# fishaudio/Bert-VITS2

Hardware: AMD Instinct MI355X
Metric: audio-seconds/sec (44.1 kHz), SynthesizerTrn.infer(), 128-phoneme utterance (higher is better)
Workload: dtype f32; 1 GPU; BASELINE config 2: B=1 x T=128 symbols per GPU, fp32 Generator (split-bf16 MFMA), fp32 flow, fp32 text encoder / durations / spline; utterances_per_gpu=1, symbols=128, frames=384, parallelism=utterance-sharded x1, hipgraph=False, hip_force_dev_kernarg=1

## Files before the change

### bert-vits2_amd/csrc/bv2_api.cpp

```cpp
#include <cmath>
#include <cstddef>
#include <cstring>
#include <functional>
#include <new>

#include "bv2_internal.h"

using namespace bv2;

static thread_local std::string g_create_err;

#define BV2_TRY try {
#define BV2_CATCH(h_)                                                                  \
  } catch (const std::exception& e) {                                                  \
    if (h_) (h_)->err = std::string("exception: ") + e.what();                         \
    return -100;                                                                       \
  } catch (...) {                                                                      \
    if (h_) (h_)->err = "unknown exception";                                           \
    return -100;                                                                       \
  }

extern "C" {

int bv2_abi_version(void) { return BV2_ABI_VERSION; }
// ... 459 lines not shown
}

int bv2_graph_num_nodes(const bv2_graph* g) { return g ? g->nodes : -1; }

void bv2_graph_destroy(bv2_graph* g) {
  if (!g) return;
  if (g->exec) (void)hipGraphExecDestroy(g->exec);
  delete g;
}

int bv2_set_option(bv2_handle* h, const char* key, int value) {
  if (!h) return -1;
  BV2_TRY
  const std::string k = key ? key : "";
  if (k == "fused_resblock") h->no_fused_resblock = value == 0;
  else if (k == "fused_respair") h->no_fused_respair = value == 0;
  else if (k == "fused_boundary") h->no_fused_boundary = value == 0;
  else if (k == "x6_pair") h->no_x6_pair = value == 0;
  else if (k == "x6_pair_c64") h->no_x6_pair_c64 = value == 0;
  else if (k == "x6_pair_c16") h->no_x6_pair_c16 = value == 0;
  else if (k == "x6_pair_c128") h->x6_pair_c128 = value != 0;
  else if (k == "respair_mix") h->respair_problem_major = value == 0;
  else if (k == "respair_form") h->respair_form = value;
  else if (k == "respair_c32") h->no_respair_c32 = value == 0;
  else if (k == "f16_wn") h->f16_wn = value;
  else if (k == "f16_ni") h->f16_ni = value;
  else if (k == "f16_kv") h->no_f16_kv = !value;
  else if (k == "stage_sum") h->no_stage_sum = !value;
  else if (k == "resblock_c16") h->no_resblock_c16 = value == 0;
  else if (k == "f16_fused_ln") h->no_f16_fused_ln = value == 0;
  else if (k == "f16_ksplit") h->no_f16_ksplit = value == 0;
  else if (k == "conv_post_rows") h->no_conv_post_rows = value == 0;
  else if (k == "ups_phase_taps") h->no_ups_phase_taps = value == 0;
  else if (k == "xcd_affine") h->no_xcd_affine = value == 0;
  else if (k == "prefetch") h->prefetch = value & 3;
  else if (k == "conv_x6") h->no_conv_x6 = value == 0;
  else if (k == "conv_x3") h->no_conv_x3 = value == 0;
  else if (k == "conv_x6_c32") h->x6_narrow = value != 0;
  else if (k == "fused_dds") h->no_fused_dds = value == 0;
  else if (k == "fused_attn_o") h->no_fused_attn_o = value == 0;
  else if (k == "attn_ksplit") h->attn_ksplit = value;
  else if (k == "overlap_dp") h->no_overlap_dp = value == 0;
  else { h->err = "bv2_set_option: unknown key '" + k + "'"; return -1; }
  return 0;
  BV2_CATCH(h)
}

int bv2_set_tap(bv2_handle* h, const char* name, float* dev_dst, int64_t cap) {
  if (!h) return -1;
  BV2_TRY
  if (!name) { h->taps.clear(); return 0; }
  if (!dev_dst || cap <= 0) { h->taps.erase(name); return 0; }
  h->taps[name] = Tap{dev_dst, cap};
  return 0;
  BV2_CATCH(h)
}

int bv2_profile_enable(bv2_handle* h, int on) {
  if (!h) return -1;
  BV2_TRY
  if (on && h->prof_pool.empty()) {
    h->prof_pool.resize(8192);
    for (auto& r : h->prof_pool) {
      if (hipEventCreate(&r.e0) != hipSuccess || hipEventCreate(&r.e1) != hipSuccess) {
        h->err = "bv2_profile_enable: hipEventCreate failed";
        return -6;
// ... 135 lines not shown
            std::memcpy(&wy[x3_w_index(j, ci, co, cin, k, 0)], &g0, 2);
            std::memcpy(&wy[x3_w_index(j, ci, co, cin, k, 1)], &g1, 2);
          }
    }
    if (w_host && hipMemcpy(wpack_dev, pk.data(), sizeof(float) * pk.size(), hipMemcpyHostToDevice) != hipSuccess) return -6;
    ConvLaunch cl;
    std::memset(&cl, 0, sizeof(cl));
    ConvProb& p = cl.p[0];
    if (cin % 32 == 0 && ksplit <= 1) {
      float* reg = wpack_dev + t_x3_off(cin, cout, k);
      if (launch_x3_zero_slots(static_cast<hipStream_t>(stream), reinterpret_cast<unsigned*>(reg), 2)) return -6;
      p.omax = reinterpret_cast<unsigned*>(reg + X3_SLOT_WORDS);
      if (x3) {
        if (nsrc != 1 || launch_absmax(static_cast<hipStream_t>(stream), x, (int64_t)B * cin * L, reinterpret_cast<unsigned*>(reg))) return -2;
        p.xmax = reinterpret_cast<const unsigned*>(reg);
        p.w3inv = reg + 2 * X3_SLOT_WORDS; p.w3 = reinterpret_cast<const uint16_t*>(reg + 2 * X3_SLOT_WORDS + X3_HDR_FLOATS);
      }
    }
    p.x[0] = x; p.x[1] = x1; p.x[2] = x2; p.nsrc = nsrc; p.in_scale = in_scale;
    p.x_bstride = (int64_t)cin * L; p.x_rstride = L; p.Lin = L;
    p.in_mask = in_mask; p.in_mask_bstride = L; p.out_mask = out_mask; p.out_mask_bstride = L;
    p.w = wpack_dev; p.bias = bias_host ? wpack_dev + boff : nullptr;
    if (x6) p.w6 = reinterpret_cast<const uint16_t*>(wpack_dev + t_x6_off(cin, cout, k));
    p.bias2 = bias2; p.bias2_bstride = cout;
    p.out = out; p.out_bstride = (int64_t)cout * L; p.out_rstride = L; p.out_tstride = 1; p.out_toff = 0;
    p.res = res; p.res_bstride = p.out_bstride; p.res_mode = res_mode;
    p.cin = cin; p.cin_pad = cin_pad; p.cout = cout; p.cout_pad = cout_pad; p.w_ld = ld; p.k = k; p.dil = dil;
    p.pad_left = pad_left < 0 ? ((k - 1) / 2) * dil : pad_left;
    p.pre_act = lrelu_slope != 0.f ? PRE_LRELU : PRE_NONE; p.slope = lrelu_slope;
    p.act = relu ? ACT_RELU : ACT_NONE; p.mask_pre = mask_pre; p.mask_post = mask_post;
    cl.nprob = 1; cl.B = B; cl.L = L; cl.ksplit = ksplit < 1 ? 1 : ksplit; cl.slab_stride = slab_stride;
    const char* vn = nullptr;
    return launch_conv1d(static_cast<hipStream_t>(stream), cl, tile, &vn);
  } catch (...) { return -100; }
}

int bv2_test_resblock_fused(void* stream, const float* x, float* out, const float* w1_host, const float* b1_host,
                            const float* w2_host, const float* b2_host, float* wpack_dev, int B, int C, int k, int dil, int L,
                            float slope) {
  try {
    const int cin_pad = t_round_up(C, 16);
    const size_t one = (size_t)bv2_test_conv_pack_floats(C, C, k), boff = (size_t)k * cin_pad * t_round_up(C, 128);
    std::vector<float> pk(2 * one, 0.f);
    const float* ws[2] = {w1_host, w2_host};
    const float* bs[2] = {b1_host, b2_host};
    for (int h = 0; h < 2; ++h) {
      for (int j = 0; j < k; ++j)
        for (int ci = 0; ci < C; ++ci)
          for (int co = 0; co < C; ++co)
            pk[h * one + (size_t)conv_w_index(j, ci, co, cin_pad, k)] = ws[h][((size_t)co * C + ci) * k + j];
      for (int co = 0; co < C; ++co) pk[h * one + boff + co] = bs[h][co];
    }
    if (hipMemcpy(wpack_dev, pk.data(), sizeof(float) * pk.size(), hipMemcpyHostToDevice) != hipSuccess) return -6;
    FusedLaunch F;
    std::memset(&F, 0, sizeof(F));
    F.nprob = 1; F.B = B; F.C = C; F.L = L; F.slope = slope;
    F.p[0].x = x; F.p[0].out = out; F.p[0].w1 = wpack_dev; F.p[0].b1 = wpack_dev + boff;
    F.p[0].w2 = wpack_dev + one; F.p[0].b2 = wpack_dev + one + boff; F.p[0].k = k; F.p[0].dil = dil;
    return launch_resblock_fused(static_cast<hipStream_t>(stream), F);
  } catch (...) { return -100; }
}

static inline uint16_t t_f2bf(float f) {
  uint32_t u;
  std::memcpy(&u, &f, 4);
  u += 0x7fffu + ((u >> 16) & 1u);
// ... 436 lines not shown
```

### bert-vits2_amd/csrc/bv2_exec.cpp

```cpp
#include <cmath>
#include <cstdlib>
#include <cstring>

#include "bv2_internal.h"

namespace bv2 {

namespace {

struct Arena {
  char* base;
  int64_t off = 0, cap;
  Arena(void* b, int64_t c) : base(static_cast<char*>(b)), cap(c) {}
  template <class T> T* get(int64_t n) {
    const int64_t bytes = (n * (int64_t)sizeof(T) + 255) / 256 * 256;
    T* p = base ? reinterpret_cast<T*>(base + off) : nullptr;
    off += bytes;
    return p;
  }
  bool ok() const { return base == nullptr || off <= cap; }
};

struct Ctx {
  bv2_handle* h;
// ... 743 lines not shown
        if (!last) {
          ConvProb r = c.prob(K.wn_res[i], P.acts, P.h, Ty);
          r.res = P.h; r.res_mode = RES_ADD; r.out_mask = ymask; r.mask_post = 1;
          cl.p[cl.nprob++] = r;
        }
        ConvProb sk = c.prob(K.wn_skip[i], P.acts, P.outacc, Ty);
        if (i > 0) { sk.res = P.outacc; sk.res_mode = RES_ADD; }
        if (last) { sk.out_mask = ymask; sk.mask_post = 1; }
        cl.p[cl.nprob++] = sk;
        c.conv(cl, "wn.res_skip");
      }
      hres = P.outacc;
    }
    {
      const std::string tn = "flow." + std::to_string(a) + ".enc";
      c.tap(tn.c_str(), hres, (int64_t)B * H * Ty);
    }
    p = c.prob(K.post, hres, x1, Ty);
    p.out_bstride = (int64_t)C * Ty; p.res = x1; p.res_bstride = (int64_t)C * Ty; p.res_mode = RES_RSUB;
    p.out_mask = ymask; p.mask_post = 1;
    c.conv1(p, B, Ty, "flow.post");
    {
      const std::string tn = "flow." + std::to_string(a) + ".z";
      c.tap(tn.c_str(), z, (int64_t)B * C * Ty);
    }
  }
}

static void gen_core(Ctx& c, const PlanB& P, const float* z, int z_rstride, const float* ymask, int B, int L, float* o,
                     const int64_t* lens) {
  const Model& m = c.m;
  const bv2_config& cf = m.cfg;
  const int C = cf.inter_channels, c0 = cf.upsample_initial_channel;
  {
    ConvProb p = c.prob(m.conv_pre, z, P.pre, L);
    p.x_bstride = (int64_t)C * z_rstride; p.x_rstride = z_rstride; p.Lin = L;
    p.in_mask = ymask; p.in_mask_bstride = z_rstride;
    p.bias2 = P.gv; p.bias2_bstride = P.gv_stride;
    c.conv1(p, B, L, "dec.conv_pre", 1, 0, lens, 1);
  }
  c.tap("dec.pre", P.pre, (int64_t)B * c0 * L);
  const float* src[3] = {P.pre, nullptr, nullptr};
  int nsrc = 1;
  int Lc = L;
  int up = 1;
  int next_slot = 0;
  int n_slots = 0;
  for (int i = 0; i < m.n_ups && !c.h->no_conv_x3 && !c.h->no_conv_x6; ++i)
    if (m.ups[i].cout % 128 == 0 && m.rb[i][0][0][0].wy_off >= 0) n_slots += 1 + 2 * m.n_rbk * m.n_rbd;
  const bool any_x3 = n_slots > 0;
  if (any_x3 && !c.rc) c.chk(launch_x3_zero_slots(c.s, P.xslots, n_slots), "dec.x3_slots");
  for (int i = 0; i < m.n_ups; ++i) {
    const UpW& U = m.ups[i];
    float* const* S = P.set[i & 1];
    float* x = S[0];
    const int Lo = Lc * U.u;
    const int nb = m.n_rbk;
    const bool rb2 = m.rb_type == 2;
    bool fused = U.cout <= 32 && nb <= 3 && !c.h->no_fused_resblock && !rb2;
    bool x6pair = !rb2 && nb <= 3 && !c.h->no_fused_resblock && !c.h->no_conv_x6 && !c.h->no_x6_pair &&
                  (U.cout == 32 || (U.cout == 16 && !c.h->no_x6_pair_c16) || (U.cout == 64 && !c.h->no_x6_pair_c64) ||
                   (U.cout == 128 && c.h->x6_pair_c128));
    for (int j = 0; j < nb && x6pair; ++j)
      for (int d = 0; d < m.n_rbd && x6pair; ++d)
        x6pair = m.rb[i][j][d][0].wx_off >= 0 && m.rb[i][j][d][1].wx_off >= 0 && m.rb[i][j][d][0].k == m.rb[i][j][d][1].k &&
                 respair_x6_supported(U.cout, cf.resblock_kernel_sizes[j], cf.resblock_dilation_sizes[j][d]);
    if (x6pair) fused = true;
    if (fused && !x6pair && c.h->x6_narrow && !c.h->no_conv_x6 && U.cout == 32 && m.rb[i][0][0][0].wx_off >= 0) fused = false;
    for (int j = 0; j < nb && fused && !x6pair; ++j)
      for (int d = 0; d < m.n_rbd; ++d)
        fused = fused && resblock_fused_supported(U.cout, cf.resblock_kernel_sizes[j], cf.resblock_dilation_sizes[j][d]);
    bool x3 = any_x3 && !rb2 && !fused && U.cout % 128 == 0;
    for (int j = 0; j < nb && x3; ++j)
      for (int d = 0; d < m.n_rbd && x3; ++d) x3 = m.rb[i][j][d][0].wy_off >= 0 && m.rb[i][j][d][1].wy_off >= 0;
    unsigned* const slot_x = x3 ? P.xslots + X3_SLOT_WORDS * next_slot++ : nullptr;
    {
      ConvLaunch cl;
      cl.nprob = U.u; cl.B = B; cl.L = Lc; cl.lens = lens; cl.len_mul = up;
      for (int ph = 0; ph < U.u; ++ph) {
        ConvProb p = c.prob(U.phase[ph], src[0], x, Lc);
        p.x[1] = src[1]; p.x[2] = src[2]; p.nsrc = nsrc; p.in_scale = 1.f / (float)nsrc;
        p.pre_act = PRE_LRELU; p.slope = 0.1f;
        p.pad_left = U.pad_left[ph];
        p.out_bstride = (int64_t)U.cout * Lo; p.out_rstride = Lo; p.out_tstride = U.u; p.out_toff = ph;
        p.omax = slot_x;
        cl.p[ph] = p;
      }
      c.conv(cl, "dec.ups");
    }
    {
      const std::string tn = "dec.ups." + std::to_string(i);
      c.tap(tn.c_str(), x, (int64_t)B * U.cout * Lo);
    }
    float* branch_out[BV2_MAX_RESBLOCK_KERNELS];
    if (rb2) {
      for (int d = 0; d < m.n_rbd; ++d) {
        ConvLaunch c1;
        c1.nprob = nb; c1.B = B; c1.L = Lo; c1.lens = lens; c1.len_mul = up * U.u;
        const bool to_cur = ((m.n_rbd - 1 - d) & 1) == 0;
        for (int jj = 0; jj < nb; ++jj) {
          const int j = nb - 1 - jj;
          float* cur = S[1 + j];
          float* tmp = S[1 + nb + j];
          const float* xin = d == 0 ? x : (to_cur ? tmp : cur);
          ConvProb p = c.prob(m.rb[i][j][d][0], xin, to_cur ? cur : tmp, Lo, cf.resblock_dilation_sizes[j][d]);
          p.pre_act = PRE_LRELU; p.slope = 0.1f;
          p.res = xin; p.res_mode = RES_ADD;
          p.w6 = (!c.h->no_conv_x6 && m.rb[i][j][d][0].wx_off >= 0) ? reinterpret_cast<const uint16_t*>(c.W(m.rb[i][j][d][0].wx_off)) : nullptr;
          c1.p[jj] = p;
        }
        c.conv(c1, "dec.resblock2.conv");
// ... 404 lines not shown
```

### bert-vits2_amd/csrc/bv2_internal.h

```cpp
#pragma once
#include <hip/hip_runtime_api.h>
#include <stdint.h>

#include <map>
#include <string>
#include <vector>

#include "../../include/bv2.h"
#include "bv2_kernels.h"

namespace bv2 {

constexpr int kAttnWindow = 4;
constexpr int kCondLayer = 2;
constexpr int kSdpLayers = 3;
constexpr int kSdpKernel = 3;
constexpr int kSdpBins = 10;
constexpr int kSdpFlowsUsed = 3;
constexpr int kDpFilter = 256;
constexpr int kDpKernel = 3;
constexpr int kFlowKernel = 5;
constexpr int kMaxLayers = 16;
constexpr int kMaxFlows = 8;
constexpr uint32_t kBlobMagic = 0x32765642u;
// ... 81 lines not shown
  int post_c = 0, post_k = 7;
  int total_up = 1;
  int64_t total_floats = 0;
  uint32_t cfg_hash = 0;
};

struct HostTensor { std::vector<float> data; std::vector<int64_t> shape; };

struct ProfileRec { hipEvent_t e0, e1; int fam; double flops, bytes; };

struct Tap { float* dst; int64_t cap; };

}

struct bv2_handle {
  bv2::Model model;
  std::map<std::string, bv2::HostTensor> tensors;
  const float* blob = nullptr;
  std::string err;
  std::map<std::string, bv2::Tap> taps;
  int gen_dtype = BV2_F32;
  int flow_dtype = BV2_F32;
  bool no_conv_x6 = false;
  bool no_conv_x3 = false;
  bool x6_narrow = true;
  bool no_fused_resblock = false;
  int prefetch = 0;
  bool no_xcd_affine = false;
  bool no_f16_fused_ln = false;
  int f16_wn = 0, f16_ni = 0;
  bool no_f16_kv = false;
  bool no_f16_ksplit = false;
  bool no_conv_post_rows = false;
  bool no_ups_phase_taps = false;
  bool no_stage_sum = true;
  bool no_resblock_c16 = false;
  bool no_respair_c32 = false;
  int respair_form = 1;
  bool respair_problem_major = false;
  bool x6_pair_c128 = false;
  bool no_x6_pair_c16 = false;
  bool no_x6_pair_c64 = false;
  bool no_x6_pair = false;
  bool no_fused_boundary = false;
  bool no_fused_respair = false;
  bool no_fused_attn_o = false;
  int attn_ksplit = -1;
  bool no_fused_dds = false;
  bool no_overlap_dp = true;
  hipStream_t side_stream = nullptr;
  hipEvent_t ev_fork = nullptr, ev_join = nullptr;
  bool prof_on = false;
  int prof_mode = 1;
  std::vector<bv2::ProfileRec> prof_pool;
  size_t prof_used = 0;
  std::vector<std::string> prof_names;
};

namespace bv2 {

int build_layout(Model& m, std::string& err);
int pack_blob(const Model& m, const std::map<std::string, HostTensor>& t, float* blob, std::string& err);
bool key_in_schema(const Model& m, const std::string& key);

int64_t workspace_bytes(const Model& m, int B, int T, int Ty);
int run_encode(bv2_handle* h, hipStream_t s, const bv2_encode_in& in, const bv2_encode_out& out, void* ws, int64_t wsb,
// ... 20 lines not shown
```

### bert-vits2_amd/csrc/bv2_kernels.h

```cpp
#pragma once
#include <hip/hip_runtime_api.h>
#include <stdint.h>
#include <map>
#include <mutex>
#include <utility>

namespace bv2 {

#if defined(__HIPCC__)
__device__ __forceinline__ bool xcd_decode(unsigned id, int per, int B, int& b, int& r) {
  const unsigned slot = id >> 3;
  b = (int)(slot / (unsigned)per) * 8 + (int)(id & 7u);
  r = (int)(slot % (unsigned)per);
  return b < B;
}
#endif
inline int xcd_grid(int B, int per) { return 8 * ((B + 7) / 8) * per; }

struct Prefetch { const void* ptr; unsigned bytes; };
constexpr int PF_BLOCKS = 128;
#if defined(__HIPCC__)
__device__ __forceinline__ void prefetch_tail(const Prefetch pf, unsigned l, unsigned j, unsigned tid, unsigned nthreads) {
  const unsigned lines = (pf.bytes + 127u) >> 7;
  const unsigned lx = (lines + 7u) >> 3;
// ... 42 lines not shown
  const float* bias2;
  int bias2_bstride;
  float* out;
  int64_t out_bstride;
  int out_rstride, out_tstride, out_toff;
  const float* res;
  int64_t res_bstride;
  const float* out_mask;
  int out_mask_bstride;
  int cin, cin_pad, cout, cout_pad, w_ld, k, dil, pad_left;
  int pre_act;  float slope;
  int act;
  int mask_pre;
  int res_mode;
  int mask_post;
  const uint16_t* w3;
  const float* w3inv;
  const unsigned* xmax;
  unsigned* omax;
};

#define BV2_MAX_PROBS 8
#define BV2_MAX_KSPLIT 8
struct ConvLaunch {
  ConvProb p[BV2_MAX_PROBS];
  int nprob;
  int B;
  int L;
  const int64_t* lens = nullptr; int len_mul = 1;
  int ksplit;
  int64_t slab_stride;
  unsigned long long* dbg = nullptr;
  Prefetch pf = {nullptr, 0};
};
void conv_set_timeline(unsigned long long* dev_buf, long long capacity_u64);
int conv_timeline_report(long long* meta, int max_launches);
unsigned long long* timeline_slice(unsigned gx, unsigned gy, unsigned gz, int tile, int ks, int cin, int L);

enum { TILE_AUTO = 0, TILE_128x128 = 1, TILE_64x128 = 2, TILE_64x64 = 3, TILE_32x128 = 4, TILE_32x256 = 5, TILE_SPLITK = 6, TILE_128x64 = 7,
       TILE_X6 = 8,
       TILE_X6_128x64 = 9, TILE_X6_128x64_LD = 10, TILE_X6_64x128 = 11, TILE_X6_32x256 = 12,
       TILE_X3 = 14 };
int launch_conv1d(hipStream_t stream, const ConvLaunch& L, int tile, const char** variant_name);
inline int64_t x6_w_index(int j, int ci, int co, int cin, int k, int plane) {
  const int64_t U = (int64_t)(cin / 16) * k, u = (int64_t)(ci / 16) * k + j;
  const int lane = (co & 31) + 32 * ((ci % 16) / 8);
  return ((((int64_t)(co >> 5) * U + u) * 3 + plane) * 64 + lane) * 8 + (ci % 8);
}
inline int64_t x6_w_elems(int cin, int cout_pad, int k) { return (int64_t)(cout_pad / 32) * (cin / 16) * k * 3 * 512; }
inline void x6_split(float v, uint16_t h[3]) {
  for (int p = 0; p < 3; ++p) {
    uint32_t u;
    __builtin_memcpy(&u, &v, 4);
    uint16_t b;
    if ((u & 0x7fffffffu) > 0x7f800000u) b = (uint16_t)((u >> 16) | 0x40u);
    else if (p == 0 && (u & 0x7fffffffu) > 0x7f7f0000u) b = (uint16_t)((u >> 16) & 0x8000u) | 0x7f7fu;
    else { u += 0x7fffu + ((u >> 16) & 1u); b = (uint16_t)(u >> 16); }
    h[p] = b;
    const uint32_t w = (uint32_t)b << 16;
    float f;
    __builtin_memcpy(&f, &w, 4);
    v -= f;
  }
}
inline int64_t x3_w_index(int j, int ci, int co, int cin, int k, int plane) {
  const int64_t U = (int64_t)(cin / 16) * k, u = (int64_t)(ci / 16) * k + j;
// ... 343 lines not shown
```

### bert-vits2_amd/csrc/kernels/conv_mfma.hip

```cpp
#include <hip/hip_runtime.h>
#include "../bv2_kernels.h"

namespace bv2 {

typedef float f32x16 __attribute__((ext_vector_type(16)));
typedef float f32x4 __attribute__((ext_vector_type(4)));

__device__ __forceinline__ unsigned* x3_slot_word(unsigned* slot) {
  return slot + X3_LINE_WORDS * (__builtin_amdgcn_s_getreg((31 << 11) | 20) & 7u);
}
__device__ __forceinline__ void x3_publish(unsigned* word, unsigned seen, float vmx, int lane) {
#pragma unroll
  for (int d = 32; d >= 1; d >>= 1) vmx = fmaxf(vmx, __shfl_xor(vmx, d));
  const unsigned bits = __float_as_uint(vmx);
  if (lane == 0 && bits > seen) __hip_atomic_fetch_max(word, bits, __ATOMIC_RELAXED, __HIP_MEMORY_SCOPE_WORKGROUP);
}

__device__ __forceinline__ float ld_off(const float* base, unsigned byte_off) {
  return *reinterpret_cast<const float*>(reinterpret_cast<const char*>(base) + byte_off);
}
__device__ __forceinline__ f32x4 ld_off4(const float* base, unsigned byte_off) {
  return *reinterpret_cast<const f32x4*>(reinterpret_cast<const char*>(base) + byte_off);
}

// ... 280 lines not shown
        }
      }
    }
    if (omax_w) x3_publish(omax_w, omax_seen, vmx, lane);
  }
  if (L.dbg && tid == 0) {
    __builtin_amdgcn_s_waitcnt(0);
    unsigned long long* d = L.dbg + 8ull * (snake_n > 0 ? (unsigned long long)blockIdx.x
                                                        : ((unsigned long long)blockIdx.z * gridDim.y + blockIdx.y) * gridDim.x + blockIdx.x);
    d[0] = ts0; d[1] = ts1; d[2] = ts2; d[3] = __builtin_amdgcn_s_memtime();
    d[4] = __builtin_amdgcn_s_getreg((31 << 11) | 4);
    d[5] = __builtin_amdgcn_s_getreg((31 << 11) | 20);
    d[6] = (unsigned long long)k; d[7] = 1;
  }
}

constexpr int SK_PD = 8;


constexpr int SK_XP = 64;
constexpr int SK_RPW = 32;
template <bool MASK, int NWV, bool LDSX>
__global__ void __launch_bounds__(64 * NWV) conv1d_splitk_kernel(const ConvLaunch L, const int mtiles, const int ntiles,
                                                                 const int per_xcd, const int total) {
  extern __shared__ __attribute__((aligned(16))) float red_raw[];
  float (*red)[32][33] = reinterpret_cast<float (*)[32][33]>(red_raw);
  const int bid = blockIdx.x;
  if (bid >= per_xcd * 8) {
    prefetch_tail(L.pf, (unsigned)bid, (unsigned)(bid - per_xcd * 8), threadIdx.x, 64 * NWV);
    return;
  }
  unsigned long long ts0 = 0, ts1 = 0, ts2 = 0;
  if (L.dbg) ts0 = __builtin_amdgcn_s_memtime();
  const int v = (bid & 7) * per_xcd + (bid >> 3);
  if (v >= total) return;
  int rem = v;
  const int nt = rem % ntiles; rem /= ntiles;
  const int z = rem % L.ksplit; rem /= L.ksplit;
  const int mt = rem % mtiles; rem /= mtiles;
  const int b = rem % L.B; rem /= L.B;
  const ConvProb P = L.p[rem];
  const int m0 = mt * 32, t0 = nt * 32;
  if (m0 >= P.cout_pad) return;

  const int tid = threadIdx.x;
  const int lane = tid & 63;
  const int wid = __builtin_amdgcn_readfirstlane(tid >> 6);
  const int l31 = lane & 31, lh = lane >> 5;
  const int k = P.k, dil = P.dil, cin = P.cin;
  int Lin = P.Lin;
  if (L.lens) {
    const int64_t lv = L.lens[b] * L.len_mul;
    Lin = lv < Lin ? (int)lv : Lin;
  }
  const int groups = P.cin_pad / 8;
  const float in_scale = P.in_scale, slope = P.slope;
  const bool lrelu = P.pre_act == PRE_LRELU;
  const float* const xp = P.x[0] + (int64_t)b * P.x_bstride;
  const float* const mp = MASK ? P.in_mask + (int64_t)b * P.in_mask_bstride : nullptr;
  const float* const wp = P.w;
  const unsigned x_rs4 = 4u * (unsigned)P.x_rstride;
  const unsigned w_tap = 1024u;
  const unsigned w_unit = w_tap * (unsigned)k;
  const unsigned w_lane = 16u * (unsigned)(lh * 32 + l31) + (unsigned)mt * (unsigned)groups * w_unit;
  const unsigned nsl = (unsigned)(L.ksplit * NWV), sl = (unsigned)(z * NWV + wid);
  const int g0 = (int)(((unsigned)groups * sl) / nsl), g1 = (int)(((unsigned)groups * (sl + 1u)) / nsl);
// ... 352 lines not shown

static int launch_splitk(hipStream_t stream, const ConvLaunch& L0, int max_cout_pad, const char** variant_name) {
  const int mtiles = max_cout_pad / 32, ntiles = (L0.L + 31) / 32;
  const ConvLaunch L = with_timeline(L0, dim3(((L0.nprob * L0.B * mtiles * L0.ksplit * ntiles + 7) / 8) * 8), 32032);
  const int total = L.nprob * L.B * mtiles * L.ksplit * ntiles;
  const int per_xcd = (total + 7) / 8;
  bool any_mask = false, all_mask = true;
  for (int i = 0; i < L.nprob; ++i) {
    if (L.p[i].nsrc != 1) return -2;
    if (L.p[i].in_mask) any_mask = true; else all_mask = false;
  }
  if (any_mask != all_mask) return -2;
  int nw = splitk_waves(L);
  for (int i = 0; i < L.nprob; ++i)
    if (L.p[i].act == ACT_GATE && nw == 16) nw = 8;
  if (variant_name) *variant_name = nw == 16 ? "conv1d_splitk<32x32,16w>" : (nw == 8 ? "conv1d_splitk<32x32,8w>" : "conv1d_splitk<32x32,4w>");
  const dim3 grid(per_xcd * 8 + (L.pf.ptr && L.pf.bytes ? PF_BLOCKS : 0));
  bool ldsx = !g_tune_no_ldsx;
  const int stage_rows = splitk_stage_rows(L, nw);
  for (int i = 0; i < L.nprob; ++i)
    if (L.p[i].k < 2 || 32 + (L.p[i].k - 1) * L.p[i].dil > SK_XP) ldsx = false;
  if (stage_rows > SK_RPW * nw) ldsx = false;
  if (variant_name && ldsx) *variant_name = nw == 16 ? "conv1d_splitk_ldsx<32x32,16w>" : (nw == 8 ? "conv1d_splitk_ldsx<32x32,8w>" : "conv1d_splitk_ldsx<32x32,4w>");
  if (ldsx) {
    if (any_mask) launch_splitk_nw<true, true>(stream, L, nw, grid, mtiles, ntiles, per_xcd, total, stage_rows);
    else launch_splitk_nw<false, true>(stream, L, nw, grid, mtiles, ntiles, per_xcd, total, stage_rows);
  } else {
    if (any_mask) launch_splitk_nw<true, false>(stream, L, nw, grid, mtiles, ntiles, per_xcd, total, stage_rows);
    else launch_splitk_nw<false, false>(stream, L, nw, grid, mtiles, ntiles, per_xcd, total, stage_rows);
  }
  return hipGetLastError() == hipSuccess ? 0 : -1;
}

int conv_pick_ksplit(const ConvLaunch& L, int max_split) {
  if (max_split <= 1) return 1;
  int groups = 1 << 30;
  for (int i = 0; i < L.nprob; ++i) {
    if (L.p[i].cin_pad / 8 < groups) groups = L.p[i].cin_pad / 8;
    if (L.p[i].act != ACT_NONE) return 1;
  }
  const int slices = (splitk_units(L) + SK_UNITS_PER_WAVE - 1) / SK_UNITS_PER_WAVE;
  int ks = 1;
  while (ks < max_split && ks * 4 < slices && groups / (ks * 2 * 4) >= 1) ks *= 2;
  return ks;
}

bool conv_use_splitk(const ConvLaunch& L) {
  int mt = 0;
  for (int i = 0; i < L.nprob; ++i)
    if (L.p[i].cout_pad / 32 > mt) mt = L.p[i].cout_pad / 32;
  for (int i = 0; i < L.nprob; ++i)
    if (L.p[i].nsrc != 1 || (L.p[i].in_mask != nullptr) != (L.p[0].in_mask != nullptr)) return false;
  const long cols = (long)L.B * L.L;
  const long tiles128 = (long)L.nprob * mt * ((L.L + 127) / 128) * L.B;
  double flops = 0;
  for (int i = 0; i < L.nprob; ++i) flops += 2.0 * L.p[i].cout * L.p[i].cin * L.p[i].k * (double)cols;
  if (flops >= 2e9 && tiles128 >= 128 && L.L >= 64) return false;
  return cols <= 4096 && tiles128 < 512;
}

int launch_conv1d(hipStream_t stream, const ConvLaunch& L, int tile, const char** variant_name) {
  if (L.nprob < 1 || L.nprob > BV2_MAX_PROBS || L.B < 1 || L.L < 1) return -1;
  int max_cout_pad = 0, max_extra = 0, ck = 32, max_chunks = 1;
  for (int i = 0; i < L.nprob; ++i) {
    const ConvProb& p = L.p[i];
    if (p.cout_pad % 32 || p.cin_pad % 16 || p.k < 1 || p.dil < 1 || p.w_ld % 128 || p.w_ld < p.cout_pad) return -1;
    if (p.cout_pad > max_cout_pad) max_cout_pad = p.cout_pad;
    if ((p.k - 1) * p.dil > max_extra) max_extra = (p.k - 1) * p.dil;
    if (p.cin_pad % 32) ck = 16;
  }
  if (g_tune_force_ck == 16) ck = 16;
  for (int i = 0; i < L.nprob; ++i)
    if (L.p[i].cin_pad / ck > max_chunks) max_chunks = L.p[i].cin_pad / ck;
  const bool auto_sk = tile == TILE_AUTO && conv_use_splitk(L);
  if (auto_sk) tile = TILE_SPLITK;
  if (tile == TILE_SPLITK) {
    if (L.ksplit < 1 || L.ksplit > BV2_MAX_KSPLIT) return -1;
    return launch_splitk(stream, L, max_cout_pad, variant_name);
  }
  if (L.ksplit != 1) return -1;
  if (tile >= TILE_X6) return launch_conv1d_x6(stream, L, tile, variant_name);
  if (tile == TILE_AUTO && g_tune_tile_target == 0 && conv_x6_supported(L)) return launch_conv1d_x6(stream, L, TILE_X6, variant_name);
  if (tile == TILE_AUTO) {
    const long target = g_tune_tile_target > 0 ? g_tune_tile_target : 1536L;
    if (((g_tune_tile_target == -7 && max_cout_pad % 128 == 0) || (g_tune_tile_target == -8 && max_cout_pad == 128)) &&
        64 + max_extra <= 128) {
      if (variant_name) *variant_name = kTile128x64.name;
      return launch_variant<2, 2, 2, 1, 2>(stream, L, ck, max_cout_pad, max_extra, max_chunks);
    }
    if ((g_tune_tile_target == -9 && max_cout_pad == 64) || (g_tune_tile_target == -10 && max_cout_pad == 128)) {
      if (variant_name) *variant_name = "conv1d_mfma<64x128>";
      return launch_variant<2, 2, 1, 2, 3>(stream, L, ck, max_cout_pad, max_extra, max_chunks);
    }
    if (g_tune_tile_target == -11 && max_cout_pad == 128) {
      if (variant_name) *variant_name = "conv1d_mfma<128x128>";
      return launch_variant<2, 2, 2, 2, 3>(stream, L, ck, max_cout_pad, max_extra, max_chunks);
    }
    tile = TILE_32x128;
    double best_score = -1.0;
    bool reached = false;
    for (const TileCfg& t : kTiles) {
      if (t.bm > max_cout_pad && t.bm != 32) continue;
      if (max_cout_pad % t.bm && t.bm != 32) continue;
      if (t.bn + max_extra > t.xs * 64) continue;
      const long nb = (L.L + t.bn - 1) / t.bn;
      const long blocks = nb * ((max_cout_pad + t.bm - 1) / t.bm) * L.B * L.nprob;
      const double useful = (double)L.L / (double)(nb * t.bn);
      if (blocks >= target && useful >= 0.75) { tile = t.id; reached = true; break; }
      const double score = (double)(blocks < target ? blocks : target) * useful;
      if (score > best_score) { best_score = score; tile = t.id; }
    }
    (void)reached;
  }
  for (const TileCfg& t : kTiles)
    if (t.id == tile && variant_name) *variant_name = t.name;
// ... 31 lines not shown
```

### include/bv2_testing.h

```cpp
#ifndef BV2_TESTING_H
#define BV2_TESTING_H
#include <stdint.h>
#include "bv2.h"
#ifdef __cplusplus
extern "C" {
#endif

int64_t bv2_test_conv_pack_floats(int cin, int cout, int k);

int bv2_test_conv1d(void* stream, const float* x, const float* w_host, const float* bias_host, float* out, float* wpack_dev,
                    int B, int cin, int cout, int k, int dil, int pad_left, int L, int tile, float lrelu_slope, int relu,
                    const float* res, int res_mode, const float* in_mask, const float* out_mask, int mask_pre,
                    int mask_post, const float* bias2, int nsrc, const float* x1, const float* x2, float in_scale, int ksplit,
                    int64_t slab_stride);


int64_t bv2_test_x3_omax_off(int cin, int cout, int k);

void bv2_test_x6_split(float v, uint16_t* h3);
int bv2_test_x6_regions(const bv2_handle* h, int64_t* off_floats, int64_t* n_floats, int max_regions);
int bv2_test_x3_regions(const bv2_handle* h, int64_t* off_floats, int64_t* n_floats, int max_regions);

int bv2_test_resblock_fused(void* stream, const float* x, float* out, const float* w1_host, const float* b1_host,
                            const float* w2_host, const float* b2_host, float* wpack_dev, int B, int C, int k, int dil, int L,
                            float slope);

int64_t bv2_test_conv_cl_pack_bytes(int cin, int cout, int k);
int bv2_test_conv_cl_bf16(void* stream, const void* x0, const void* x1, const void* x2, int nsrc, const float* w_host,
                          const float* bias_host, void* wpack_dev, void* out, const void* res, const float* bias2, int B, int cin,
                          int cout, int k, int dil, int pad_left, int L, int pre_lrelu, float slope);

int64_t bv2_test_resblock_cl_pack_bytes(int C, int k, int nd);
int bv2_test_resblock_cl(void* stream, const void* x, void* out, const float* w_host, const float* bias_host, void* wpack_dev, int B,
                         int C, int k, const int* dil, int nd, int L, float slope, int variant, const int64_t* lens);

int64_t bv2_test_respair_cl_pack_bytes(int C, int k);
int bv2_test_respair_cl(void* stream, const void* x, void* out, const float* w_host, const float* bias_host, void* wpack_dev, int B,
                        int C, int k, int dil, int L, float slope, int form, const int64_t* lens);
int64_t bv2_test_respair_x6_pack_bytes(int C, int k);
int bv2_test_respair_x6(void* stream, const float* x, float* out, const float* w_host, const float* bias_host, void* wpack_dev, int B,
                        int C, int k, int dil, int L, float slope, const int64_t* lens);
int bv2_test_respair_x3(void* stream, const float* x, float* out, const float* w_host, const float* bias_host, void* wpack_dev, int B,
                        int C, int k, int dil, int L, float slope, const int64_t* lens);
int64_t bv2_test_flow_boundary_pack_floats(int C);
int bv2_test_flow_boundary(void* stream, const float* a, int nslab, int64_t slab_stride, const float* gamma, const float* beta,
                           const float* mask, float* x1, int64_t z_bstride, const float* post_w_host, const float* post_b_host,
                           const float* pre_w_host, const float* pre_b_host, float* pre_out, float* wpack_dev, int B, int C, int T);

int bv2_test_conv_f16(void* stream, const void* x, int in_ct, const float* in_mask, const float* w_host, const float* bias_host,
                      void* wpack_dev, void* out, int out_ct, const float* res, int res_mode, const float* out_mask, int mask_pre,
                      int mask_post, int act, int B, int cin, int cout, int k, int dil, int L, int out_rstride);

int bv2_test_dump_cl_conv(bv2_handle* h, const void* host_blob, int kind, int i, int j, int d, int e, int32_t* dims,
                          float* w_out, float* bias_out);
// ... 34 lines not shown
```

Baseline: 1465 audio-seconds/sec.

## Merge upsample phases into one MFMA kernel and fold slot zeroing into conv_pre

Adds a dedicated kernel that computes all u polyphase sub-convolutions of a transposed-conv upsample in one block. It stages the input tile in LDS once, shares it across phases, and writes the interleaved phases with a single vector store per lane. It is enabled by default only for single-tap stages (ups_merged=1). Separately, zeroing of the x3 max slots is folded into the split-K conv_pre launch, which removes a small separate kernel launch. The risks are higher register pressure from U accumulators and losing the previously tuned generic or x6 tile paths for those stages.

```diff
diff --git a/bert-vits2_amd/csrc/bv2_api.cpp b/bert-vits2_amd/csrc/bv2_api.cpp
--- a/bert-vits2_amd/csrc/bv2_api.cpp
+++ b/bert-vits2_amd/csrc/bv2_api.cpp
@@ -515,6 +515,7 @@
   else if (k == "f16_ksplit") h->no_f16_ksplit = value == 0;
   else if (k == "conv_post_rows") h->no_conv_post_rows = value == 0;
   else if (k == "ups_phase_taps") h->no_ups_phase_taps = value == 0;
+  else if (k == "ups_merged") h->ups_merged = value < 0 ? 0 : (value > 2 ? 2 : value);
   else if (k == "xcd_affine") h->no_xcd_affine = value == 0;
   else if (k == "prefetch") h->prefetch = value & 3;
   else if (k == "conv_x6") h->no_conv_x6 = value == 0;
@@ -716,6 +717,58 @@
     cl.nprob = 1; cl.B = B; cl.L = L; cl.ksplit = ksplit < 1 ? 1 : ksplit; cl.slab_stride = slab_stride;
     const char* vn = nullptr;
     return launch_conv1d(static_cast<hipStream_t>(stream), cl, tile, &vn);
+  } catch (...) { return -100; }
+}
+
+static int64_t t_ups_region(int cin, int cout, int nt) { return t_x6_off(cin, cout, nt); }
+int64_t bv2_test_ups_omax_off(int cin, int cout, int u, int k) { return u < 1 ? -1 : (int64_t)u * t_ups_region(cin, cout, k / u); }
+int64_t bv2_test_ups_pack_floats(int cin, int cout, int u, int k) { return bv2_test_ups_omax_off(cin, cout, u, k) + X3_SLOT_WORDS; }
+int bv2_test_ups(void* stream, const float* x0, const float* x1, const float* x2, int nsrc, const float* w_host, const float* bias_host,
+                 float* out, float* wpack_dev, int B, int cin, int cout, int u, int k, int L, const int64_t* lens, int len_mul, float slope,
+                 int form) {
+  try {
+    if (u < 1 || u > BV2_MAX_PROBS || k < u || k % u || (k - u) % 2 || nsrc < 1 || nsrc > 3 || !w_host || !x0 || !out || !wpack_dev) return -1;
+    if (form != 0 && form != 1) return -2;
+    const int nt = k / u, pad = (k - u) / 2;
+    const int cin_pad = t_round_up(cin, 16), ld = t_round_up(cout, 128), cout_pad = t_round_up(cout, 32);
+    const int64_t region = t_ups_region(cin, cout, nt);
+    const size_t boff = (size_t)nt * cin_pad * ld;
+    std::vector<float> pk((size_t)region * u, 0.f);
+    int pad_left[BV2_MAX_PROBS];
+    for (int ph = 0; ph < u; ++ph) {
+      const int pp = (ph + pad) % u, shift = (ph + pad) / u;
+      pad_left[ph] = (nt - 1) - shift;
+      float* r = pk.data() + (size_t)region * ph;
+      for (int j = 0; j < nt; ++j)
+        for (int ci = 0; ci < cin; ++ci)
+          for (int co = 0; co < cout; ++co)
+            r[(size_t)conv_w_index(j, ci, co, cin_pad, nt)] = w_host[((size_t)ci * cout + co) * k + pp + u * (nt - 1 - j)];
+      if (bias_host) for (int co = 0; co < cout; ++co) r[boff + co] = bias_host[co];
+    }
+    if (hipMemcpy(wpack_dev, pk.data(), sizeof(float) * pk.size(), hipMemcpyHostToDevice) != hipSuccess) return -6;
+    unsigned* const slot = reinterpret_cast<unsigned*>(wpack_dev + bv2_test_ups_omax_off(cin, cout, u, k));
+    if (launch_x3_zero_slots(static_cast<hipStream_t>(stream), slot, 1)) return -6;
+    const int Lo = L * u;
+    ConvLaunch cl;
+    std::memset(&cl, 0, sizeof(cl));
+    cl.nprob = u; cl.B = B; cl.L = L; cl.lens = lens; cl.len_mul = len_mul < 1 ? 1 : len_mul; cl.ksplit = 1;
+    cl.ups_merged = form == 1 ? 1 : 0;
+    for (int ph = 0; ph < u; ++ph) {
+      ConvProb& p = cl.p[ph];
+      p.x[0] = x0; p.x[1] = nsrc > 1 ? x1 : nullptr; p.x[2] = nsrc > 2 ? x2 : nullptr; p.nsrc = nsrc; p.in_scale = 1.f / (float)nsrc;
+      p.x_bstride = (int64_t)cin * L; p.x_rstride = L; p.Lin = L;
+      p.in_mask_bstride = L; p.out_mask_bstride = L;
+      p.w = wpack_dev + region * ph; p.bias = bias_host ? p.w + boff : nullptr;
+      p.out = out; p.out_bstride = (int64_t)cout * Lo; p.out_rstride = Lo; p.out_tstride = u; p.out_toff = ph;
+      p.res_bstride = p.out_bstride;
+      p.cin = cin; p.cin_pad = cin_pad; p.cout = cout; p.cout_pad = cout_pad; p.w_ld = ld; p.k = nt; p.dil = 1; p.pad_left = pad_left[ph];
+      p.pre_act = PRE_LRELU; p.slope = slope;
+      p.omax = slot;
+    }
+    const char* vn = "";
+    const int rc = launch_conv1d(static_cast<hipStream_t>(stream), cl, TILE_AUTO, &vn);
+    if (rc) return rc < 0 ? rc : -rc;
+    return vn && std::strncmp(vn, "ups_merged", 10) == 0 ? 1 : 0;
   } catch (...) { return -100; }
 }
 
diff --git a/bert-vits2_amd/csrc/bv2_exec.cpp b/bert-vits2_amd/csrc/bv2_exec.cpp
--- a/bert-vits2_amd/csrc/bv2_exec.cpp
+++ b/bert-vits2_amd/csrc/bv2_exec.cpp
@@ -799,12 +799,21 @@
   const Model& m = c.m;
   const bv2_config& cf = m.cfg;
   const int C = cf.inter_channels, c0 = cf.upsample_initial_channel;
+  int n_slots = 0;
+  for (int i = 0; i < m.n_ups && !c.h->no_conv_x3 && !c.h->no_conv_x6; ++i)
+    if (m.ups[i].cout % 128 == 0 && m.rb[i][0][0][0].wy_off >= 0) n_slots += 1 + 2 * m.n_rbk * m.n_rbd;
+  const bool any_x3 = n_slots > 0;
+  bool slots_by_pre = false;
   {
     ConvProb p = c.prob(m.conv_pre, z, P.pre, L);
     p.x_bstride = (int64_t)C * z_rstride; p.x_rstride = z_rstride; p.Lin = L;
     p.in_mask = ymask; p.in_mask_bstride = z_rstride;
     p.bias2 = P.gv; p.bias2_bstride = P.gv_stride;
-    c.conv1(p, B, L, "dec.conv_pre", 1, 0, lens, 1);
+    ConvLaunch cl;
+    cl.p[0] = p; cl.nprob = 1; cl.B = B; cl.L = L; cl.lens = lens; cl.len_mul = 1;
+    slots_by_pre = any_x3 && conv_use_splitk(cl);
+    if (slots_by_pre) { cl.zero = P.xslots; cl.zero_n = n_slots * X3_SLOT_WORDS; }
+    c.conv(cl, "dec.conv_pre");
   }
   c.tap("dec.pre", P.pre, (int64_t)B * c0 * L);
   const float* src[3] = {P.pre, nullptr, nullptr};
@@ -812,11 +821,7 @@
   int Lc = L;
   int up = 1;
   int next_slot = 0;
-  int n_slots = 0;
-  for (int i = 0; i < m.n_ups && !c.h->no_conv_x3 && !c.h->no_conv_x6; ++i)
-    if (m.ups[i].cout % 128 == 0 && m.rb[i][0][0][0].wy_off >= 0) n_slots += 1 + 2 * m.n_rbk * m.n_rbd;
-  const bool any_x3 = n_slots > 0;
-  if (any_x3 && !c.rc) c.chk(launch_x3_zero_slots(c.s, P.xslots, n_slots), "dec.x3_slots");
+  if (any_x3 && !slots_by_pre && !c.rc) c.chk(launch_x3_zero_slots(c.s, P.xslots, n_slots), "dec.x3_slots");
   for (int i = 0; i < m.n_ups; ++i) {
     const UpW& U = m.ups[i];
     float* const* S = P.set[i & 1];
@@ -844,6 +849,7 @@
     {
       ConvLaunch cl;
       cl.nprob = U.u; cl.B = B; cl.L = Lc; cl.lens = lens; cl.len_mul = up;
+      cl.ups_merged = c.h->ups_merged >= 2 || (c.h->ups_merged == 1 && U.ntaps == 1);
       for (int ph = 0; ph < U.u; ++ph) {
         ConvProb p = c.prob(U.phase[ph], src[0], x, Lc);
         p.x[1] = src[1]; p.x[2] = src[2]; p.nsrc = nsrc; p.in_scale = 1.f / (float)nsrc;
diff --git a/bert-vits2_amd/csrc/bv2_internal.h b/bert-vits2_amd/csrc/bv2_internal.h
--- a/bert-vits2_amd/csrc/bv2_internal.h
+++ b/bert-vits2_amd/csrc/bv2_internal.h
@@ -137,6 +137,7 @@
   bool no_f16_kv = false;
   bool no_f16_ksplit = false;
   bool no_conv_post_rows = false;
+  int ups_merged = 1;
   bool no_ups_phase_taps = false;
   bool no_stage_sum = true;
   bool no_resblock_c16 = false;
diff --git a/bert-vits2_amd/csrc/bv2_kernels.h b/bert-vits2_amd/csrc/bv2_kernels.h
--- a/bert-vits2_amd/csrc/bv2_kernels.h
+++ b/bert-vits2_amd/csrc/bv2_kernels.h
@@ -98,6 +98,8 @@
   int64_t slab_stride;
   unsigned long long* dbg = nullptr;
   Prefetch pf = {nullptr, 0};
+  int ups_merged = 0;
+  unsigned* zero = nullptr; int zero_n = 0;
 };
 void conv_set_timeline(unsigned long long* dev_buf, long long capacity_u64);
 int conv_timeline_report(long long* meta, int max_launches);
diff --git a/bert-vits2_amd/csrc/kernels/conv_mfma.hip b/bert-vits2_amd/csrc/kernels/conv_mfma.hip
--- a/bert-vits2_amd/csrc/kernels/conv_mfma.hip
+++ b/bert-vits2_amd/csrc/kernels/conv_mfma.hip
@@ -336,6 +336,8 @@
   }
   unsigned long long ts0 = 0, ts1 = 0, ts2 = 0;
   if (L.dbg) ts0 = __builtin_amdgcn_s_memtime();
+  if (L.zero)
+    for (int i = bid * (64 * NWV) + (int)threadIdx.x; i < L.zero_n; i += per_xcd * 8 * (64 * NWV)) L.zero[i] = 0u;
   const int v = (bid & 7) * per_xcd + (bid >> 3);
   if (v >= total) return;
   int rem = v;
@@ -754,6 +756,280 @@
   return hipGetLastError() == hipSuccess ? 0 : -1;
 }
 
+template <int U, int WM, int WN, int CK, int XS>
+__global__ void __launch_bounds__(64 * WM * WN) ups_merged_kernel(const ConvLaunch L, const int mtiles, const int per_xcd, const int pad_max) {
+  constexpr int NW = WM * WN;
+  constexpr int BM = WM * 32;
+  constexpr int BN = WN * 32;
+  constexpr int XP = XS * 64 + 32;
+  constexpr int RPW = CK / NW;
+  constexpr int GR = CK / 8;
+  static_assert(U == 2 || U == 4, "phases per lane: one 8- or 16-byte store");
+  static_assert(CK % NW == 0, "whole rows per wave");
+  extern __shared__ __attribute__((aligned(16))) float smem[];
+
+  const ConvProb P = L.p[0];
+  const int tid = threadIdx.x;
+  const int lane = tid & 63;
+  const int wid = __builtin_amdgcn_readfirstlane(tid >> 6);
+  const int l31 = lane & 31, lh = lane >> 5;
+  const int wm = wid / WN, wn = wid % WN;
+  unsigned long long ts0 = 0, ts1 = 0, ts2 = 0;
+  if (L.dbg) ts0 = __builtin_amdgcn_s_memtime();
+  const int by = blockIdx.y, bx = blockIdx.x;
+  const int b = by / mtiles;
+  const int m0 = (by - b * mtiles) * BM;
+  const int vt = per_xcd ? (bx & 7) * per_xcd + (bx >> 3) : bx;
+  const int t0 = vt * BN;
+  if (t0 >= L.L) return;
+
+  const int k = P.k, cin = P.cin, nsrc = P.nsrc;
+  int Lin = P.Lin;
+  if (L.lens) {
+    const int64_t lv = L.lens[b] * L.len_mul;
+    Lin = lv < Lin ? (int)lv : Lin;
+    if (t0 >= Lin) return;
+  }
+  const float in_scale = P.in_scale, slope = P.slope;
+  const bool lrelu = P.pre_act == PRE_LRELU;
+  const float* const x0p = P.x[0] + (int64_t)b * P.x_bstride;
+  const float* const x1p = P.x[1] ? P.x[1] + (int64_t)b * P.x_bstride : nullptr;
+  const float* const x2p = P.x[2] ? P.x[2] + (int64_t)b * P.x_bstride : nullptr;
+  const int x_rstride = P.x_rstride;
+  const int nchunks = P.cin_pad / CK;
+  const int groups = P.cin_pad / 8;
+  float* Xs = smem;
+
+  const int mt = (m0 >> 5) + wm;
+  const float* wq[U];
+  unsigned xsh[U];
+  const float* biasq[U];
+#pragma unroll
+  for (int ph = 0; ph < U; ++ph) {
+    wq[ph] = L.p[ph].w + (int64_t)mt * groups * k * 256;
+    xsh[ph] = 4u * (unsigned)(pad_max - L.p[ph].pad_left);
+    biasq[ph] = L.p[ph].bias;
+  }
+  const unsigned wlane = 16u * (unsigned)lane;
+
+  f32x16 acc[U];
+#pragma unroll
+  for (int ph = 0; ph < U; ++ph)
+#pragma unroll
+    for (int r = 0; r < 16; ++r) acc[ph][r] = 0.f;
+
+  float xr[RPW][XS];
+  const int tbase = t0 - pad_max;
+  unsigned tc[XS];
+  float colsc[XS];
+#pragma unroll
+  for (int s = 0; s < XS; ++s) {
+    const int t = tbase + lane + 64 * s;
+    const bool tok = t >= 0 && t < Lin;
+    colsc[s] = tok ? in_scale : 0.f;
+    tc[s] = 4u * (unsigned)(t < 0 ? 0 : (t >= Lin ? Lin - 1 : t));
+  }
+  auto issue_x = [&](int c) __attribute__((always_inline)) {
+    unsigned roff[RPW];
+#pragma unroll
+    for (int r = 0; r < RPW; ++r) {
+      int cg = c * CK + wid * RPW + r;
+      cg = cg < cin ? cg : cin - 1;
+      roff[r] = 4u * (unsigned)cg * (unsigned)x_rstride;
+    }
+#pragma unroll
+    for (int s = 0; s < XS; ++s)
+#pragma unroll
+      for (int r = 0; r < RPW; ++r) xr[r][s] = ld_off(x0p, roff[r] + tc[s]);
+    if (nsrc > 1) {
+      __builtin_amdgcn_sched_barrier(0);
+#pragma unroll
+      for (int s = 0; s < XS; ++s)
+#pragma unroll
+        for (int r = 0; r < RPW; ++r) xr[r][s] += ld_off(x1p, roff[r] + tc[s]);
+      if (nsrc > 2) {
+        __builtin_amdgcn_sched_barrier(0);
+#pragma unroll
+        for (int s = 0; s < XS; ++s)
+#pragma unroll
+          for (int r = 0; r < RPW; ++r) xr[r][s] += ld_off(x2p, roff[r] + tc[s]);
+      }
+    }
+  };
+  auto store_x = [&](int c, int buf) __attribute__((always_inline)) {
+    float* dst = Xs + buf * (CK * XP) + (wid * RPW) * XP + lane;
+    const int rows_ok = cin - (c * CK + wid * RPW);
+#pragma unroll
+    for (int s = 0; s < XS; ++s) {
+      const float sc = colsc[s] * 1.f;
+#pragma unroll
+      for (int r = 0; r < RPW; ++r) {
+        float v = xr[r][s];
+        const float vn = v * slope;
+        v = (lrelu && v < 0.f) ? vn : v;
+        v *= sc;
+        dst[r * XP + 64 * s] = r < rows_ok ? v : 0.f;
+      }
+    }
+  };
+  auto load_w = [&](f32x4 (&a)[U][GR], int c, int j) __attribute__((always_inline)) {
+#pragma unroll
+    for (int ph = 0; ph < U; ++ph)
+#pragma unroll
+      for (int g = 0; g < GR; ++g) a[ph][g] = ld_off4(wq[ph] + ((int64_t)(c * GR + g) * k + j) * 256, wlane);
+  };
+
+  unsigned* const omax_w = P.omax ? x3_slot_word(P.omax) : nullptr;
+  unsigned omax_seen = 0xffffffffu;
+  if (omax_w) omax_seen = *reinterpret_cast<volatile unsigned*>(omax_w);
+  f32x4 aw[U][GR];
+  issue_x(0);
+  load_w(aw, 0, 0);
+  const int cout = P.cout, Lout = L.L;
+  const unsigned o_rs = (unsigned)P.out_rstride;
+  float* const outb = P.out + (int64_t)b * P.out_bstride;
+  const int row0 = m0 + wm * 32 + 4 * lh;
+  store_x(0, 0);
+  omax_seen = __builtin_amdgcn_readfirstlane(omax_seen);
+  __syncthreads();
+  if (L.dbg) ts1 = __builtin_amdgcn_s_memtime();
+
+  const unsigned xlane = 4u * (unsigned)(lh * XP + wn * 32 + l31);
+  const char* const xs_bytes = reinterpret_cast<const char*>(Xs);
+  for (int c = 0; c < nchunks; ++c) {
+    const bool next_chunk = (c + 1) < nchunks;
+    if (next_chunk) issue_x(c + 1);
+    const unsigned xbuf = xlane + (unsigned)(c & 1) * (unsigned)(CK * XP * 4);
+    for (int j = 0; j < k; ++j) {
+      const unsigned xcol = xbuf + 4u * (unsigned)j;
+#pragma unroll
+      for (int g = 0; g < GR; ++g)
+#pragma unroll
+        for (int q = 0; q < 4; ++q)
+#pragma unroll
+          for (int ph = 0; ph < U; ++ph) {
+            const float bv = *reinterpret_cast<const float*>(xs_bytes + xcol + xsh[ph] + 4 * ((8 * g + 2 * q) * XP));
+            const float a = q == 0 ? aw[ph][g].x : (q == 1 ? aw[ph][g].y : (q == 2 ? aw[ph][g].z : aw[ph][g].w));
+            acc[ph] = __builtin_amdgcn_mfma_f32_32x32x2f32(a, bv, acc[ph], 0, 0, 0);
+          }
+      if (next_chunk || j + 1 < k) load_w(aw, j + 1 == k ? c + 1 : c, j + 1 == k ? 0 : j + 1);
+    }
+    if (next_chunk) {
+      store_x(c + 1, (c + 1) & 1);
+      __syncthreads();
+    }
+  }
+
+  if (L.dbg) ts2 = __builtin_amdgcn_s_memtime();
+  {
+    const int col = t0 + wn * 32 + l31;
+    const bool colok = col < Lout;
+    const unsigned off0 = (unsigned)row0 * o_rs + (unsigned)(colok ? col : 0) * (unsigned)U;
+    float bs[U][16];
+#pragma unroll
+    for (int ph = 0; ph < U; ++ph) {
+      const float* const b1p = biasq[ph] ? biasq[ph] : wq[ph];
+      const unsigned m_b1 = biasq[ph] ? 0xffffffffu : 0u;
+#pragma unroll
+      for (int r = 0; r < 16; ++r) {
+        int row = row0 + (r & 3) + 8 * (r >> 2);
+        row = row < cout ? row : cout - 1;
+        bs[ph][r] = __uint_as_float(__float_as_uint(ld_off(b1p, m_b1 ? 4u * (unsigned)row : 0u)) & m_b1);
+      }
+    }
+    float vmx = 0.f;
+#pragma unroll
+    for (int r = 0; r < 16; ++r) {
+      const int dr = (r & 3) + 8 * (r >> 2);
+      float v[U];
+#pragma unroll
+      for (int ph = 0; ph < U; ++ph) v[ph] = acc[ph][r] + (bs[ph][r] + 0.f);
+      if (colok && row0 + dr < cout) {
+        float* const dst = outb + off0 + (unsigned)dr * o_rs;
+        if constexpr (U == 2) {
+          typedef float f32x2 __attribute__((ext_vector_type(2)));
+          f32x2 o; o.x = v[0]; o.y = v[1];
+          *reinterpret_cast<f32x2*>(dst) = o;
+        } else {
+          f32x4 o; o.x = v[0]; o.y = v[1]; o.z = v[2]; o.w = v[3];
+          *reinterpret_cast<f32x4*>(dst) = o;
+        }
+#pragma unroll
+        for (int ph = 0; ph < U; ++ph) vmx = fmaxf(vmx, fabsf(v[ph]));
+      }
+    }
+    if (omax_w) x3_publish(omax_w, omax_seen, vmx, lane);
+  }
+  if (L.dbg && tid == 0) {
+    __builtin_amdgcn_s_waitcnt(0);
+    unsigned long long* d = L.dbg + 8ull * ((unsigned long long)blockIdx.y * gridDim.x + blockIdx.x);
+    d[0] = ts0; d[1] = ts1; d[2] = ts2; d[3] = __builtin_amdgcn_s_memtime();
+    d[4] = __builtin_amdgcn_s_getreg((31 << 11) | 4);
+    d[5] = __builtin_amdgcn_s_getreg((31 << 11) | 20);
+    d[6] = (unsigned long long)k; d[7] = 1;
+  }
+}
+
+static bool ups_merged_covers(const ConvLaunch& L, int* pad_max_out, int* span_out) {
+  const int u = L.nprob;
+  if ((u != 2 && u != 4) || L.ksplit != 1) return false;
+  const ConvProb& a = L.p[0];
+  int pmax = a.pad_left, pmin = a.pad_left;
+  for (int i = 0; i < u; ++i) {
+    const ConvProb& p = L.p[i];
+    if (p.out_tstride != u || p.out_toff != i || p.dil != 1 || p.act != ACT_NONE || p.res_mode != RES_NONE || p.in_mask || p.out_mask ||
+        p.bias2 || p.w6 || p.pad_left < 0)
+      return false;
+    if (p.x[0] != a.x[0] || p.x[1] != a.x[1] || p.x[2] != a.x[2] || p.nsrc != a.nsrc || p.in_scale != a.in_scale ||
+        p.x_bstride != a.x_bstride || p.x_rstride != a.x_rstride || p.Lin != a.Lin || p.out != a.out || p.out_bstride != a.out_bstride ||
+        p.out_rstride != a.out_rstride || p.cin != a.cin || p.cin_pad != a.cin_pad || p.cout != a.cout || p.cout_pad != a.cout_pad ||
+        p.w_ld != a.w_ld || p.k != a.k || p.pre_act != a.pre_act || p.slope != a.slope || p.omax != a.omax || (p.bias != nullptr) != (a.bias != nullptr))
+      return false;
+    pmax = p.pad_left > pmax ? p.pad_left : pmax;
+    pmin = p.pad_left < pmin ? p.pad_left : pmin;
+  }
+  if (reinterpret_cast<uintptr_t>(a.out) % (4u * u) || a.out_rstride % u || a.out_bstride % u) return false;
+  if (a.nsrc < 1 || a.nsrc > 3 || (a.nsrc > 1 && !a.x[1]) || (a.nsrc > 2 && !a.x[2])) return false;
+  if ((int64_t)a.cout_pad * a.out_rstride >= (1ll << 31) || (int64_t)a.cin * a.x_rstride >= (1ll << 29)) return false;
+  *pad_max_out = pmax;
+  *span_out = (a.k - 1) + (pmax - pmin);
+  return *span_out <= 64;
+}
+
+template <int U, int WM, int WN, int XS>
+static int launch_ups_merged_t(hipStream_t stream, const ConvLaunch& L0, int ck, int pad_max) {
+  constexpr int BM = WM * 32, BN = WN * 32;
+  const int mtiles = L0.p[0].cout_pad / BM;
+  const int ntx = (L0.L + BN - 1) / BN;
+  const int per_xcd = (ntx % 8 == 0 || ntx >= 64) ? (ntx + 7) / 8 : 0;
+  const dim3 grid(per_xcd ? per_xcd * 8 : ntx, mtiles * L0.B, 1);
+  const ConvLaunch L = with_timeline(L0, grid, 900000 + U * 10000 + BM * 10 + WN);
+  const int nxbuf = L0.p[0].cin_pad / ck > 1 ? 2 : 1;
+  const size_t lds = sizeof(float) * (size_t)(nxbuf * ck * (XS * 64 + 32));
+  if (ck == 32) hipLaunchKernelGGL((ups_merged_kernel<U, WM, WN, 32, XS>), grid, dim3(64 * WM * WN), lds, stream, L, mtiles, per_xcd, pad_max);
+  else hipLaunchKernelGGL((ups_merged_kernel<U, WM, WN, 16, XS>), grid, dim3(64 * WM * WN), lds, stream, L, mtiles, per_xcd, pad_max);
+  return hipGetLastError() == hipSuccess ? 0 : -1;
+}
+
+template <int U>
+static int launch_ups_merged(hipStream_t stream, const ConvLaunch& L, int ck, int pad_max, int span, const char** variant_name) {
+  const int cout_pad = L.p[0].cout_pad;
+  const long target = 512;
+  const long wg22 = cout_pad % 64 == 0 ? (long)((L.L + 63) / 64) * (cout_pad / 64) * L.B : 0;
+  const long wg14 = (long)((L.L + 127) / 128) * (cout_pad / 32) * L.B;
+  const int force = g_tune_tile_target <= -21 && g_tune_tile_target >= -23 ? (int)-g_tune_tile_target - 20 : 0;
+  if (force ? (force == 1 && wg22 > 0) : wg22 >= target) {
+    if (variant_name) *variant_name = "ups_merged<64x64>";
+    return span ? launch_ups_merged_t<U, 2, 2, 2>(stream, L, ck, pad_max) : launch_ups_merged_t<U, 2, 2, 1>(stream, L, ck, pad_max);
+  }
+  if (force ? force == 2 : wg14 >= target / 2) {
+    if (variant_name) *variant_name = "ups_merged<32x128>";
+    return span ? launch_ups_merged_t<U, 1, 4, 3>(stream, L, ck, pad_max) : launch_ups_merged_t<U, 1, 4, 2>(stream, L, ck, pad_max);
+  }
+  if (variant_name) *variant_name = "ups_merged<32x64>";
+  return span ? launch_ups_merged_t<U, 1, 2, 2>(stream, L, ck, pad_max) : launch_ups_merged_t<U, 1, 2, 1>(stream, L, ck, pad_max);
+}
+
 int conv_pick_ksplit(const ConvLaunch& L, int max_split) {
   if (max_split <= 1) return 1;
   int groups = 1 << 30;
@@ -800,9 +1076,16 @@
     if (L.ksplit < 1 || L.ksplit > BV2_MAX_KSPLIT) return -1;
     return launch_splitk(stream, L, max_cout_pad, variant_name);
   }
+  if (L.zero) return -1;
   if (L.ksplit != 1) return -1;
   if (tile >= TILE_X6) return launch_conv1d_x6(stream, L, tile, variant_name);
   if (tile == TILE_AUTO && g_tune_tile_target == 0 && conv_x6_supported(L)) return launch_conv1d_x6(stream, L, TILE_X6, variant_name);
+  if (tile == TILE_AUTO && (g_tune_tile_target == 0 || g_tune_tile_target <= -21) && L.ups_merged) {
+    int pad_max = 0, span = 0;
+    if (ups_merged_covers(L, &pad_max, &span))
+      return L.nprob == 2 ? launch_ups_merged<2>(stream, L, ck, pad_max, span, variant_name)
+                          : launch_ups_merged<4>(stream, L, ck, pad_max, span, variant_name);
+  }
   if (tile == TILE_AUTO) {
     const long target = g_tune_tile_target > 0 ? g_tune_tile_target : 1536L;
     if (((g_tune_tile_target == -7 && max_cout_pad % 128 == 0) || (g_tune_tile_target == -8 && max_cout_pad == 128)) &&
diff --git a/include/bv2_testing.h b/include/bv2_testing.h
--- a/include/bv2_testing.h
+++ b/include/bv2_testing.h
@@ -20,6 +20,12 @@
 void bv2_test_x6_split(float v, uint16_t* h3);
 int bv2_test_x6_regions(const bv2_handle* h, int64_t* off_floats, int64_t* n_floats, int max_regions);
 int bv2_test_x3_regions(const bv2_handle* h, int64_t* off_floats, int64_t* n_floats, int max_regions);
+
+int64_t bv2_test_ups_pack_floats(int cin, int cout, int u, int k);
+int64_t bv2_test_ups_omax_off(int cin, int cout, int u, int k);
+int bv2_test_ups(void* stream, const float* x0, const float* x1, const float* x2, int nsrc, const float* w_host, const float* bias_host,
+                 float* out, float* wpack_dev, int B, int cin, int cout, int u, int k, int L, const int64_t* lens, int len_mul, float slope,
+                 int form);
 
 int bv2_test_resblock_fused(void* stream, const float* x, float* out, const float* w1_host, const float* b1_host,
                             const float* w2_host, const float* b2_host, float* wpack_dev, int B, int C, int k, int dil, int L,
```

New measurement: 1456 audio-seconds/sec. No clear change (-0.6%).
